# Enigmatisms/cvx_proj

Measured on AMD Instinct MI355X. Metric: local homographies/sec + Mpix/sec warp, 4K pair 200x200 mesh, higher is better.
Workload: dtype f64; 1 GPU; C3: 3840x2160 pair, 2000 correspondences, 200x200 mesh, canvas 4009x2242; mode=pairs, variant=auto, launch=eager, parallelism=pairsx1

## Files before the change

cvx_proj_amd/csrc/apap_kernels.hip:

```cpp
#include <hip/hip_runtime.h>

#include <cstdlib>
#include <type_traits>
#include <vector>

#include "apap_internal.h"
#include "apap_warp_dev.h"
#include "apap_weight_dev.h"

namespace {

using apap::inv3;
using apap::rcp_full;

using apap::kMoments;
constexpr int kWave = 64;

struct BatchStride {
    long long table, vertices, moments, denorm, H;
};


constexpr int kExpBits = 9;
constexpr int kExpN = 1 << kExpBits;
constexpr double kExpScale = (double)kExpN * 0x1.71547652b82fep+0;
__constant__ double kExp2Tab[kExpN] = {
    0x1.0000000000000p+0, 0x1.0058c86da1c0ap+0, 0x1.00b1afa5abcbfp+0, 0x1.010ab5b2cbd11p+0,
    0x1.0163da9fb3335p+0, 0x1.01bd1e77170b4p+0, 0x1.02168143b0281p+0, 0x1.027003103b10ep+0,
    0x1.02c9a3e778061p+0, 0x1.032363d42b027p+0, 0x1.037d42e11bbccp+0, 0x1.03d7411915a8ap+0,
    0x1.04315e86e7f85p+0, 0x1.048b9b35659d8p+0, 0x1.04e5f72f654b1p+0, 0x1.0540727fc1762p+0,
    0x1.059b0d3158574p+0, 0x1.05f5c74f0bec2p+0, 0x1.0650a0e3c1f89p+0, 0x1.06ab99fa6407cp+0,
    0x1.0706b29ddf6dep+0, 0x1.0761ead925493p+0, 0x1.07bd42b72a836p+0, 0x1.0818ba42e7d30p+0,
    0x1.0874518759bc8p+0, 0x1.08d0088f8093fp+0, 0x1.092bdf66607e0p+0, 0x1.0987d61701716p+0,
    0x1.09e3ecac6f383p+0, 0x1.0a402331b9715p+0, 0x1.0a9c79b1f3919p+0, 0x1.0af8f03834e52p+0,
    0x1.0b5586cf9890fp+0, 0x1.0bb23d833d93fp+0, 0x1.0c0f145e46c85p+0, 0x1.0c6c0b6bdae53p+0,
    0x1.0cc922b7247f7p+0, 0x1.0d265a4b520bap+0, 0x1.0d83b23395decp+0, 0x1.0de12a7b26300p+0,
    0x1.0e3ec32d3d1a2p+0, 0x1.0e9c7c55189c6p+0, 0x1.0efa55fdfa9c5p+0, 0x1.0f58503328e6dp+0,
    0x1.0fb66affed31bp+0, 0x1.1014a66f951cep+0, 0x1.1073028d7233ep+0, 0x1.10d17f64d9ef1p+0,
    0x1.11301d0125b51p+0, 0x1.118edb6db2dc1p+0, 0x1.11edbab5e2ab6p+0, 0x1.124cbae51a5c8p+0,
    0x1.12abdc06c31ccp+0, 0x1.130b1e264a0e9p+0, 0x1.136a814f204abp+0, 0x1.13ca058cbae1ep+0,
    0x1.1429aaea92de0p+0, 0x1.1489717425438p+0, 0x1.14e95934f312ep+0, 0x1.154962388149ep+0,
    0x1.15a98c8a58e51p+0, 0x1.1609d83606e12p+0, 0x1.166a45471c3c2p+0, 0x1.16cad3c92df73p+0,
    0x1.172b83c7d517bp+0, 0x1.178c554eaea89p+0, 0x1.17ed48695bbc0p+0, 0x1.184e5d23816c9p+0,
    0x1.18af9388c8deap+0, 0x1.1910eba4df41fp+0, 0x1.1972658375d2fp+0, 0x1.19d4013041dc2p+0,
    0x1.1a35beb6fcb75p+0, 0x1.1a979e2363cf8p+0, 0x1.1af99f8138a1cp+0, 0x1.1b5bc2dc40bf0p+0,
    0x1.1bbe084045cd4p+0, 0x1.1c206fb91588fp+0, 0x1.1c82f95281c6bp+0, 0x1.1ce5a51860746p+0,
    0x1.1d4873168b9aap+0, 0x1.1dab6358e15e8p+0, 0x1.1e0e75eb44027p+0, 0x1.1e71aad999e82p+0,
    0x1.1ed5022fcd91dp+0, 0x1.1f387bf9cda38p+0, 0x1.1f9c18438ce4dp+0, 0x1.1fffd7190241ep+0,
    0x1.2063b88628cd6p+0, 0x1.20c7bc96ffc18p+0, 0x1.212be3578a819p+0, 0x1.21902cd3d09b9p+0,
    0x1.21f49917ddc96p+0, 0x1.2259282fc1f27p+0, 0x1.22bdda27912d1p+0, 0x1.2322af0b63bffp+0,
    0x1.2387a6e756238p+0, 0x1.23ecc1c78903ap+0, 0x1.2451ffb82140ap+0, 0x1.24b760c547f15p+0,
    0x1.251ce4fb2a63fp+0, 0x1.25828c65fa1ffp+0, 0x1.25e85711ece75p+0, 0x1.264e450b3cb82p+0,
    0x1.26b4565e27cddp+0, 0x1.271a8b16f0a30p+0, 0x1.2780e341ddf29p+0, 0x1.27e75eeb3ab98p+0,
    0x1.284dfe1f56381p+0, 0x1.28b4c0ea83f36p+0, 0x1.291ba7591bb70p+0, 0x1.2982b17779965p+0,
    0x1.29e9df51fdee1p+0, 0x1.2a5130f50d65cp+0, 0x1.2ab8a66d10f13p+0, 0x1.2b203fc675d1fp+0,
    0x1.2b87fd0dad990p+0, 0x1.2befde4f2e280p+0, 0x1.2c57e39771b2fp+0, 0x1.2cc00cf2f6c18p+0,
    0x1.2d285a6e4030bp+0, 0x1.2d90cc15d5346p+0, 0x1.2df961f641589p+0, 0x1.2e621c1c14833p+0,
    0x1.2ecafa93e2f56p+0, 0x1.2f33fd6a454d2p+0, 0x1.2f9d24abd886bp+0, 0x1.300670653dfe4p+0,
    0x1.306fe0a31b715p+0, 0x1.30d975721b004p+0, 0x1.31432edeeb2fdp+0, 0x1.31ad0cf63eeacp+0,
    0x1.32170fc4cd831p+0, 0x1.3281375752b40p+0, 0x1.32eb83ba8ea32p+0, 0x1.3355f4fb45e20p+0,
    0x1.33c08b26416ffp+0, 0x1.342b46484ebb4p+0, 0x1.3496266e3fa2dp+0, 0x1.35012ba4ea77dp+0,
    0x1.356c55f929ff1p+0, 0x1.35d7a577dd72bp+0, 0x1.36431a2de883bp+0, 0x1.36aeb428335b4p+0,
    0x1.371a7373aa9cbp+0, 0x1.3786581d3f669p+0, 0x1.37f26231e754ap+0, 0x1.385e91be9c811p+0,
    0x1.38cae6d05d866p+0, 0x1.393761742d808p+0, 0x1.39a401b7140efp+0, 0x1.3a10c7a61d55bp+0,
    0x1.3a7db34e59ff7p+0, 0x1.3aeac4bcdf3eap+0, 0x1.3b57fbfec6cf4p+0, 0x1.3bc559212ef89p+0,
    0x1.3c32dc313a8e5p+0, 0x1.3ca0853c10f28p+0, 0x1.3d0e544ede173p+0, 0x1.3d7c4976d27fap+0,
    0x1.3dea64c123422p+0, 0x1.3e58a63b0a09bp+0, 0x1.3ec70df1c5175p+0, 0x1.3f359bf29743fp+0,
    0x1.3fa4504ac801cp+0, 0x1.40132b07a35dfp+0, 0x1.40822c367a024p+0, 0x1.40f153e4a136ap+0,
    0x1.4160a21f72e2ap+0, 0x1.41d016f44d8f5p+0, 0x1.423fb2709468ap+0, 0x1.42af74a1af3f1p+0,
    0x1.431f5d950a897p+0, 0x1.438f6d5817663p+0, 0x1.43ffa3f84b9d4p+0, 0x1.4470018321a1ap+0,
    0x1.44e086061892dp+0, 0x1.4551318eb43ecp+0, 0x1.45c2042a7d232p+0, 0x1.4632fde7006f4p+0,
    0x1.46a41ed1d0057p+0, 0x1.471566f8827d0p+0, 0x1.4786d668b3237p+0, 0x1.47f86d3001fe5p+0,
    0x1.486a2b5c13cd0p+0, 0x1.48dc10fa920a1p+0, 0x1.494e1e192aed2p+0, 0x1.49c052c5916c4p+0,
    0x1.4a32af0d7d3dep+0, 0x1.4aa532feaada6p+0, 0x1.4b17dea6db7d7p+0, 0x1.4b8ab213d5283p+0,
    0x1.4bfdad5362a27p+0, 0x1.4c70d073537cap+0, 0x1.4ce41b817c114p+0, 0x1.4d578e8bb586bp+0,
    0x1.4dcb299fddd0dp+0, 0x1.4e3eeccbd7b2ap+0, 0x1.4eb2d81d8abffp+0, 0x1.4f26eba2e35f0p+0,
    0x1.4f9b2769d2ca7p+0, 0x1.500f8b804f127p+0, 0x1.508417f4531eep+0, 0x1.50f8ccd3deb0dp+0,
    0x1.516daa2cf6642p+0, 0x1.51e2b00da3b14p+0, 0x1.5257de83f4eefp+0, 0x1.52cd359dfd53dp+0,
    0x1.5342b569d4f82p+0, 0x1.53b85df598d78p+0, 0x1.542e2f4f6ad27p+0, 0x1.54a4298571b06p+0,
    0x1.551a4ca5d920fp+0, 0x1.559098bed1bdfp+0, 0x1.56070dde910d2p+0, 0x1.567dac1351819p+0,
    0x1.56f4736b527dap+0, 0x1.576b63f4d854cp+0, 0x1.57e27dbe2c4cfp+0, 0x1.5859c0d59ca07p+0,
    0x1.58d12d497c7fdp+0, 0x1.5948c32824135p+0, 0x1.59c0827ff07ccp+0, 0x1.5a386b5f43d92p+0,
    0x1.5ab07dd485429p+0, 0x1.5b28b9ee20d1ep+0, 0x1.5ba11fba87a03p+0, 0x1.5c19af482fc8fp+0,
    0x1.5c9268a5946b7p+0, 0x1.5d0b4be135accp+0, 0x1.5d84590998b93p+0, 0x1.5dfd902d47c65p+0,
    0x1.5e76f15ad2148p+0, 0x1.5ef07ca0cbf0fp+0, 0x1.5f6a320dceb71p+0, 0x1.5fe411b078d26p+0,
    0x1.605e1b976dc09p+0, 0x1.60d84fd15612ap+0, 0x1.6152ae6cdf6f4p+0, 0x1.61cd3778bc944p+0,
    0x1.6247eb03a5585p+0, 0x1.62c2c91c56acdp+0, 0x1.633dd1d1929fdp+0, 0x1.63b90532205d8p+0,
    0x1.6434634ccc320p+0, 0x1.64afec30678b7p+0, 0x1.652b9febc8fb7p+0, 0x1.65a77e8dcc390p+0,
    0x1.6623882552225p+0, 0x1.669fbcc140be7p+0, 0x1.671c1c70833f6p+0, 0x1.6798a7420a036p+0,
    0x1.68155d44ca973p+0, 0x1.68923e87bfb7ap+0, 0x1.690f4b19e9538p+0, 0x1.698c830a4c8d4p+0,
    0x1.6a09e667f3bcdp+0, 0x1.6a877541ee718p+0, 0x1.6b052fa75173ep+0, 0x1.6b8315a736c75p+0,
    0x1.6c012750bdabfp+0, 0x1.6c7f64b30aa09p+0, 0x1.6cfdcddd47645p+0, 0x1.6d7c62dea2f8ap+0,
    0x1.6dfb23c651a2fp+0, 0x1.6e7a10a38cee8p+0, 0x1.6ef9298593ae5p+0, 0x1.6f786e7ba9fefp+0,
    0x1.6ff7df9519484p+0, 0x1.70777ce1303f6p+0, 0x1.70f7466f42e87p+0, 0x1.71773c4eaa988p+0,
    0x1.71f75e8ec5f74p+0, 0x1.7277ad3ef9011p+0, 0x1.72f8286ead08ap+0, 0x1.7378d02d50b8fp+0,
    0x1.73f9a48a58174p+0, 0x1.747aa5953c849p+0, 0x1.74fbd35d7cbfdp+0, 0x1.757d2df29ce7cp+0,
    0x1.75feb564267c9p+0, 0x1.768069c1a861dp+0, 0x1.77024b1ab6e09p+0, 0x1.7784597eeba8fp+0,
    0x1.780694fde5d3fp+0, 0x1.7888fda749e5dp+0, 0x1.790b938ac1cf6p+0, 0x1.798e56b7fcf03p+0,
    0x1.7a11473eb0187p+0, 0x1.7a94652e958aap+0, 0x1.7b17b0976cfdbp+0, 0x1.7b9b2988fb9ecp+0,
    0x1.7c1ed0130c132p+0, 0x1.7ca2a4456e7a3p+0, 0x1.7d26a62ff86f0p+0, 0x1.7daad5e2850acp+0,
    0x1.7e2f336cf4e62p+0, 0x1.7eb3bedf2e1b9p+0, 0x1.7f3878491c491p+0, 0x1.7fbd5fbab091fp+0,
    0x1.80427543e1a12p+0, 0x1.80c7b8f4abaa9p+0, 0x1.814d2add106d9p+0, 0x1.81d2cb0d1736ap+0,
    0x1.82589994cce13p+0, 0x1.82de968443d9ap+0, 0x1.8364c1eb941f7p+0, 0x1.83eb1bdadb46dp+0,
    0x1.8471a4623c7adp+0, 0x1.84f85b91e07f1p+0, 0x1.857f4179f5b21p+0, 0x1.8606562ab00ecp+0,
    0x1.868d99b4492edp+0, 0x1.87150c27004c2p+0, 0x1.879cad931a436p+0, 0x1.88247e08e1957p+0,
    0x1.88ac7d98a6699p+0, 0x1.8934ac52be8f7p+0, 0x1.89bd0a478580fp+0, 0x1.8a4597875c644p+0,
    0x1.8ace5422aa0dbp+0, 0x1.8b574029db01ep+0, 0x1.8be05bad61778p+0, 0x1.8c69a6bdb5598p+0,
    0x1.8cf3216b5448cp+0, 0x1.8d7ccbc6c19e6p+0, 0x1.8e06a5e0866d9p+0, 0x1.8e90afc931857p+0,
    0x1.8f1ae99157736p+0, 0x1.8fa553499284bp+0, 0x1.902fed0282c8ap+0, 0x1.90bab6ccce12cp+0,
    0x1.9145b0b91ffc6p+0, 0x1.91d0dad829e70p+0, 0x1.925c353aa2fe2p+0, 0x1.92e7bff148396p+0,
    0x1.93737b0cdc5e5p+0, 0x1.93ff669e2802bp+0, 0x1.948b82b5f98e5p+0, 0x1.9517cf65253d1p+0,
    0x1.95a44cbc8520fp+0, 0x1.9630faccf9243p+0, 0x1.96bdd9a7670b3p+0, 0x1.974ae95cba768p+0,
    0x1.97d829fde4e50p+0, 0x1.98659b9bddb5bp+0, 0x1.98f33e47a22a2p+0, 0x1.9981121235681p+0,
    0x1.9a0f170ca07bap+0, 0x1.9a9d4d47f2598p+0, 0x1.9b2bb4d53fe0dp+0, 0x1.9bba4dc5a3dd3p+0,
    0x1.9c49182a3f090p+0, 0x1.9cd81414380f2p+0, 0x1.9d674194bb8d5p+0, 0x1.9df6a0bcfc15ep+0,
    0x1.9e86319e32323p+0, 0x1.9f15f4499c647p+0, 0x1.9fa5e8d07f29ep+0, 0x1.a0360f4424fcbp+0,
    0x1.a0c667b5de565p+0, 0x1.a156f23701b15p+0, 0x1.a1e7aed8eb8bbp+0, 0x1.a2789dacfe68cp+0,
    0x1.a309bec4a2d33p+0, 0x1.a39b1231475f7p+0, 0x1.a42c980460ad8p+0, 0x1.a4be504f696b1p+0,
    0x1.a5503b23e255dp+0, 0x1.a5e25893523d4p+0, 0x1.a674a8af46052p+0, 0x1.a7072b8950a73p+0,
    0x1.a799e1330b358p+0, 0x1.a82cc9be14dcap+0, 0x1.a8bfe53c12e59p+0, 0x1.a95333beb0b7ep+0,
    0x1.a9e6b5579fdbfp+0, 0x1.aa7a6a1897fd2p+0, 0x1.ab0e521356ebap+0, 0x1.aba26d59a09eep+0,
    0x1.ac36bbfd3f37ap+0, 0x1.accb3e100301ep+0, 0x1.ad5ff3a3c2774p+0, 0x1.adf4dcca5a413p+0,
    0x1.ae89f995ad3adp+0, 0x1.af1f4a17a4735p+0, 0x1.afb4ce622f2ffp+0, 0x1.b04a868742ee4p+0,
    0x1.b0e07298db666p+0, 0x1.b17692a8fa8cdp+0, 0x1.b20ce6c9a8952p+0, 0x1.b2a36f0cf3f3ap+0,
    0x1.b33a2b84f15fbp+0, 0x1.b3d11c43bbd62p+0, 0x1.b468415b749b1p+0, 0x1.b4ff9ade433c6p+0,
    0x1.b59728de5593ap+0, 0x1.b62eeb6ddfc87p+0, 0x1.b6c6e29f1c52ap+0, 0x1.b75f0e844bfc6p+0,
    0x1.b7f76f2fb5e47p+0, 0x1.b89004b3a7804p+0, 0x1.b928cf22749e4p+0, 0x1.b9c1ce8e77680p+0,
    0x1.ba5b030a1064ap+0, 0x1.baf46ca7a67a7p+0, 0x1.bb8e0b79a6f1fp+0, 0x1.bc27df9285775p+0,
    0x1.bcc1e904bc1d2p+0, 0x1.bd5c27e2cb5e5p+0, 0x1.bdf69c3f3a207p+0, 0x1.be91462c95b60p+0,
    0x1.bf2c25bd71e09p+0, 0x1.bfc73b0468d30p+0, 0x1.c06286141b33dp+0, 0x1.c0fe06ff301f4p+0,
    0x1.c199bdd85529cp+0, 0x1.c235aab23e61ep+0, 0x1.c2d1cd9fa652cp+0, 0x1.c36e26b34e065p+0,
    0x1.c40ab5fffd07ap+0, 0x1.c4a77b9881650p+0, 0x1.c544778fafb22p+0, 0x1.c5e1a9f8630adp+0,
    0x1.c67f12e57d14bp+0, 0x1.c71cb269e601fp+0, 0x1.c7ba88988c933p+0, 0x1.c8589584661a1p+0,
    0x1.c8f6d9406e7b5p+0, 0x1.c99553dfa8313p+0, 0x1.ca3405751c4dbp+0, 0x1.cad2ee13da7cbp+0,
    0x1.cb720dcef9069p+0, 0x1.cc1164b994d23p+0, 0x1.ccb0f2e6d1675p+0, 0x1.cd50b869d8f0fp+0,
    0x1.cdf0b555dc3fap+0, 0x1.ce90e9be12cb9p+0, 0x1.cf3155b5bab74p+0, 0x1.cfd1f95018d17p+0,
    0x1.d072d4a07897cp+0, 0x1.d113e7ba2c38cp+0, 0x1.d1b532b08c968p+0, 0x1.d256b596f948cp+0,
    0x1.d2f87080d89f2p+0, 0x1.d39a638197a3cp+0, 0x1.d43c8eacaa1d6p+0, 0x1.d4def2158a91fp+0,
    0x1.d5818dcfba487p+0, 0x1.d62461eec14bep+0, 0x1.d6c76e862e6d3p+0, 0x1.d76ab3a99745bp+0,
    0x1.d80e316c98398p+0, 0x1.d8b1e7e2d479dp+0, 0x1.d955d71ff6075p+0, 0x1.d9f9ff37adb4ap+0,
    0x1.da9e603db3285p+0, 0x1.db42fa45c4dfdp+0, 0x1.dbe7cd63a8315p+0, 0x1.dc8cd9ab294e4p+0,
    0x1.dd321f301b460p+0, 0x1.ddd79e065807dp+0, 0x1.de7d5641c0658p+0, 0x1.df2347f63c159p+0,
    0x1.dfc97337b9b5fp+0, 0x1.e06fd81a2ece1p+0, 0x1.e11676b197d17p+0, 0x1.e1bd4f11f8220p+0,
    0x1.e264614f5a129p+0, 0x1.e30bad7dcee90p+0, 0x1.e3b333b16ee12p+0, 0x1.e45af3fe592e8p+0,
    0x1.e502ee78b3ff6p+0, 0x1.e5ab2334ac7eep+0, 0x1.e653924676d76p+0, 0x1.e6fc3bc24e350p+0,
    0x1.e7a51fbc74c83p+0, 0x1.e84e3e4933c7ep+0, 0x1.e8f7977cdb740p+0, 0x1.e9a12b6bc3181p+0,
    0x1.ea4afa2a490dap+0, 0x1.eaf503ccd2be5p+0, 0x1.eb9f4867cca6ep+0, 0x1.ec49c80faa594p+0,
    0x1.ecf482d8e67f1p+0, 0x1.ed9f78d802dc2p+0, 0x1.ee4aaa2188510p+0, 0x1.eef616ca06dd6p+0,
    0x1.efa1bee615a27p+0, 0x1.f04da28a52e59p+0, 0x1.f0f9c1cb6412ap+0, 0x1.f1a61cbdf5be7p+0,
    0x1.f252b376bba97p+0, 0x1.f2ff860a70c22p+0, 0x1.f3ac948dd7274p+0, 0x1.f459df15b82acp+0,
    0x1.f50765b6e4540p+0, 0x1.f5b5288633625p+0, 0x1.f6632798844f8p+0, 0x1.f7116302bd526p+0,
    0x1.f7bfdad9cbe14p+0, 0x1.f86e8f32a4b45p+0, 0x1.f91d802243c89p+0, 0x1.f9ccadbdac61dp+0,
    0x1.fa7c1819e90d8p+0, 0x1.fb2bbf4c0ba54p+0, 0x1.fbdba3692d514p+0, 0x1.fc8bc4866e8adp+0,
    0x1.fd3c22b8f71f1p+0, 0x1.fdecbe15f6314p+0, 0x1.fe9d96b2a23d9p+0, 0x1.ff4eaca4391b6p+0};

__device__ __forceinline__ double exp_neg_scaled(double yu, const double *tab ) {
    constexpr double L = 0x1.62e42fefa39efp-1 / kExpN;
    const int nk = (int)(-yu);
    const double f = __builtin_amdgcn_fract(yu);
    const double t = tab[nk & (kExpN - 1)];
    double p = fma(f, L * L * L * L / 24, -(L * L * L / 6));
    p = fma(f, p, L * L / 2);
    p = fma(f, p, -L);
    p = fma(f, p, 1.0);
    return __builtin_ldexp(t * p, nk >> kExpBits);
}

__device__ __forceinline__ double cell_weight_sq_tab(double vx, double vy, double sx, double sy,
                                                     double scaled_inv_sigma2, double gamma2, const double *tab) {
    const double dx = vx - sx;
    const double dy = vy - sy;
    const double x = fma(dx, dx, fma(dy, dy, 1e-300));
    const double y = __builtin_amdgcn_rsq(x);
    double g = x * y;
    const double e = fma(-g, y, 1.0);
    const double c = fma(e, 0.375, 0.5);
    g = fma(g * e, c, g);
    return fmax(exp_neg_scaled(g * scaled_inv_sigma2, tab), gamma2);
}

__device__ __forceinline__ double cell_weight_sq_f32(float vx, float vy, float2 s, float neg_scale, float gamma2) {
    const float dx = vx - s.x;
    const float dy = vy - s.y;
    const float d = __builtin_amdgcn_sqrtf(__builtin_fmaf(dx, dx, dy * dy));
    return (double)fmaxf(__builtin_amdgcn_exp2f(d * neg_scale), gamma2);
}

constexpr double kGammaCutF64 = 0x1p128;
__host__ __device__ inline double k1_gamma2(double gamma, bool w32) {
    if (gamma >= (w32 ? 1.0 : kGammaCutF64)) return 1.0;
    return gamma > 0.0 ? gamma * gamma : 0.0;
}

constexpr double kTraceFloorF64 = 1e-280;
constexpr double kTraceFloorW32 = 0x1p-40;

constexpr long long kTable24Marker = 0x7ff8242424242424ll;
__device__ __forceinline__ bool table_is_24(const double *__restrict__ table) {
    return __double_as_longlong(table[28]) == kTable24Marker;
}

typedef double double4_t __attribute__((ext_vector_type(4)));
constexpr int kChunk = 64;
static_assert(kChunk % 16 == 0 && kChunk % 4 == 0, "chunk must split evenly over 256 threads and 4-keypoint steps");

struct K1Block {
    int p_begin, p_end, nchunks;
    __device__ __forceinline__ K1Block(const double *__restrict__ &table, const double *__restrict__ &vertices,
                                       const BatchStride &bs, int n, int split, int pts_per_split) {
        table += (long long)blockIdx.z * bs.table;
        vertices += (long long)blockIdx.z * bs.vertices;
        p_begin = min(n, split * pts_per_split);
        p_end = min(n, p_begin + pts_per_split);
        nchunks = (p_end - p_begin + kChunk - 1) / kChunk;
    }
};

__device__ __forceinline__ double2 cell_vertex(const double *__restrict__ vertices, int cell, int cells) {
    const int cc = min(cell, cells - 1);
    return make_double2(vertices[2 * cc], vertices[2 * cc + 1]);
}

template <int kThreads>
__device__ __forceinline__ void exp_table_copy(double *s_exp2, int tid) {
    for (int j = tid; j < kExpN; j += kThreads) s_exp2[j] = kExp2Tab[j];
}
template <int kThreads>
struct ExpTableStage {
    static_assert(kExpN % kThreads == 0 || kThreads % kExpN == 0, "exp table vs block size");
    static constexpr int kPerThread = (kExpN + kThreads - 1) / kThreads;
    double v[kPerThread];
    __device__ __forceinline__ void fetch(int tid) {
#pragma unroll
        for (int i = 0; i < kPerThread; ++i) v[i] = kExp2Tab[(tid + i * kThreads) & (kExpN - 1)];
    }
    __device__ __forceinline__ void publish(double *s_exp2, int tid) const {
#pragma unroll
        for (int i = 0; i < kPerThread; ++i) s_exp2[(tid + i * kThreads) & (kExpN - 1)] = v[i];
    }
};

__host__ __device__ constexpr int lds_off(int r, int c) { return r * 256 + ((c ^ ((r & 1) << 4)) << 3); }
#define APAP_LDS_PIECE_OFF(r, slot) ((r) * 256 + ((slot) ^ (((r) & 1) << 3)) * 16)
constexpr bool lds_swizzles_agree() {
    for (int r = 0; r < 2; ++r)
        for (int slot = 0; slot < 16; ++slot)
            if (APAP_LDS_PIECE_OFF(r, slot) != lds_off(r, 2 * slot) || APAP_LDS_PIECE_OFF(r, slot) + 8 != lds_off(r, 2 * slot + 1))
                return false;
    return true;
}
static_assert(lds_swizzles_agree(), "a staged piece lands where lds_off looks for its two columns, for both row parities");

template <int kThreads>
using ChunkStage = double2[kChunk * 16 / kThreads];
template <int kThreads>
__device__ __forceinline__ void chunk_load(ChunkStage<kThreads> &stage, const double *__restrict__ table, int tid, int first_row,
                                           int end_row) {
#pragma unroll
    for (int i = 0; i < kChunk * 16 / kThreads; ++i) {
        const int q = tid + kThreads * i;
        const int p = first_row + (q >> 4);
        stage[i] = (p < end_row) ? *reinterpret_cast<const double2 *>(table + (size_t)p * APAP_TABLE_STRIDE + 2 * (q & 15))
                                 : make_double2(0.0, 0.0);
    }
}
#define APAP_CHUNK_STORE(kThreads, buf, stage, tid)                                          \
    do {                                                                                     \
        _Pragma("unroll") for (int i_ = 0; i_ < kChunk * 16 / (kThreads); ++i_) {            \
            const int q_ = (tid) + (kThreads) * i_;                                          \
            const int r_ = q_ >> 4, slot_ = q_ & 15;                                         \
            *reinterpret_cast<double2 *>(&(buf)[APAP_LDS_PIECE_OFF(r_, slot_)]) = (stage)[i_]; \
        }                                                                                    \
    } while (0)

template <bool kW32>
struct CellWeight {
    static constexpr int kXyColumn = kW32 ? 29 : 30;
    using Xy = std::conditional_t<kW32, float2, double2>;
    double vx, vy, scaled_inv_sigma2, gamma2;
    float vxf, vyf, neg_scale_f, gamma2f;
    const double *exp2;
    __device__ __forceinline__ void set(double2 v, double inv_sigma2, double gamma2_, const double *s_exp2) {
        vx = v.x, vy = v.y;
        scaled_inv_sigma2 = inv_sigma2 * kExpScale;
        gamma2 = gamma2_;
        vxf = (float)vx, vyf = (float)vy;
        neg_scale_f = (float)(inv_sigma2 * -0x1.71547652b82fep+0), gamma2f = (float)gamma2;
        exp2 = s_exp2;
    }
    static __device__ __forceinline__ Xy read(const unsigned char *at) { return *reinterpret_cast<const Xy *>(at); }
    __device__ __forceinline__ double sq(Xy s) const {
        if constexpr (kW32) return cell_weight_sq_f32(vxf, vyf, s, neg_scale_f, gamma2f);
        else return cell_weight_sq_tab(vx, vy, s.x, s.y, scaled_inv_sigma2, gamma2, exp2);
    }
    __device__ __forceinline__ double sq(const unsigned char *at) const { return sq(read(at)); }
};

template <bool kM24>
struct Sums16 {
    double4_t acc0 = {0.0, 0.0, 0.0, 0.0}, acc1 = {0.0, 0.0, 0.0, 0.0};
    double acc_a = 0.0, acc_b = 0.0;
    __device__ __forceinline__ void step(double w2, const unsigned char *at0, const unsigned char *at1) {
        const double b0 = *reinterpret_cast<const double *>(at0);
        const double b1 = *reinterpret_cast<const double *>(at1);
        acc0 = __builtin_amdgcn_mfma_f64_16x16x4f64(w2, b0, acc0, 0, 0, 0);
        if constexpr (kM24) {
            acc_a = __builtin_amdgcn_mfma_f64_4x4x4f64(w2, b1, acc_a, 0, 0, 0);
            acc_b = __builtin_amdgcn_mfma_f64_4x4x4f64(w2, *reinterpret_cast<const double *>(at1 + 32), acc_b, 0, 0, 0);
        } else {
            acc1 = __builtin_amdgcn_mfma_f64_16x16x4f64(w2, b1, acc1, 0, 0, 0);
        }
    }
    __device__ __forceinline__ void step(double w2, double b0, double b1, double b1b) {
        acc0 = __builtin_amdgcn_mfma_f64_16x16x4f64(w2, b0, acc0, 0, 0, 0);
        if constexpr (kM24) {
            acc_a = __builtin_amdgcn_mfma_f64_4x4x4f64(w2, b1, acc_a, 0, 0, 0);
            acc_b = __builtin_amdgcn_mfma_f64_4x4x4f64(w2, b1b, acc_b, 0, 0, 0);
        } else {
            acc1 = __builtin_amdgcn_mfma_f64_16x16x4f64(w2, b1, acc1, 0, 0, 0);
        }
    }
};

struct K1Pairs {
    int pairs, splits, tiles;
};
__host__ __device__ inline void k1_unit(const K1Pairs &pp, int i, int &tile, int &split, bool &paired) {
    const int base = pp.pairs / pp.splits, rem = pp.pairs % pp.splits;
    paired = i < pp.pairs;
    if (paired) {
        split = i % pp.splits;
        tile = 2 * (i / pp.splits);
        return;
    }
    int k = i - pp.pairs;
    const int n1 = pp.tiles - 2 * (base + 1), n0 = pp.tiles - 2 * base;
    if (k < rem * n1) {
        split = k / n1;
        tile = 2 * (base + 1) + k % n1;
    } else {
        k -= rem * n1;
        split = rem + k / n0;
        tile = 2 * base + k % n0;
    }
}

__host__ __device__ constexpr int d16_cell(int lane, int i) { return (lane >> 4) + 4 * i; }
__host__ __device__ constexpr int d16_column(int lane) { return lane & 15; }
__host__ __device__ constexpr int d4_cell(int lane) { return 4 * ((lane >> 2) & 3) + (lane >> 4); }
__host__ __device__ constexpr int d4_column(int lane) { return lane & 3; }

constexpr int kLinePitch = 144;
constexpr int kLineStageBytes = 32 * kLinePitch;
__host__ __device__ constexpr int line_stage_off(int column, int cell) { return column * kLinePitch + cell * 8; }
__host__ __device__ constexpr int line_column(int lane, int j) { return 8 * j + (lane >> 3); }
__host__ __device__ constexpr int line_cell(int lane) { return 2 * (lane & 7); }
__host__ __device__ constexpr int line_stores(int sums) { return (sums + 7) / 8; }
template <int kSums>
constexpr bool line_layout_covers() {
    static_assert(kSums == 30 || kSums == 24, "the two tables");
    int staged[32][16] = {}, stored[32][16] = {};
    for (int lane = 0; lane < 64; ++lane) {
        for (int i = 0; i < 4; ++i) {
            ++staged[d16_column(lane)][d16_cell(lane, i)];
            if (kSums == 30) ++staged[16 + d16_column(lane)][d16_cell(lane, i)];
        }
        if (kSums == 24) {
            ++staged[16 + d4_column(lane)][d4_cell(lane)];
            ++staged[20 + d4_column(lane)][d4_cell(lane)];
        }
        for (int j = 0; j < line_stores(kSums); ++j) {
            const int c = line_column(lane, j);
            if (c >= 32 || line_cell(lane) + 1 >= 16 || line_stage_off(c, line_cell(lane)) % 16 != 0 ||
                line_stage_off(c, line_cell(lane) + 1) != line_stage_off(c, line_cell(lane)) + 8)
                return false;
            if (c < kSums) ++stored[c][line_cell(lane)], ++stored[c][line_cell(lane) + 1];
        }
    }
    for (int c = 0; c < 32; ++c)
        for (int cell = 0; cell < 16; ++cell)
            if (staged[c][cell] != (c < (kSums == 30 ? 32 : 24)) || stored[c][cell] != (c < kSums)) return false;
    return true;
}
static_assert(line_layout_covers<30>() && line_layout_covers<24>(),
              "the line layout stores every sum of a 16-cell group once, columns from kSums on never, from what the D layouts staged");
static_assert(kLinePitch % 16 == 0 && 16 * 8 <= kLinePitch && 4 * kLineStageBytes <= 2 * kChunk * 256,
              "16-byte reads of whole rows; four waves' stages fit the two chunk buffers");

typedef double double2_t __attribute__((ext_vector_type(2)));
__device__ __forceinline__ void slab_store_line(double *p, double2_t v) {
    asm volatile("global_store_dwordx4 %0, %1, off sc1\n\ts_nop 1" ::"v"(p), "v"(v) : "memory");
}

__global__ __launch_bounds__(256) void k_assemble_valu(const double *__restrict__ table, int n,
                                                       const double *__restrict__ vertices, int cells,
                                                       int cells_pad, double gamma2, double inv_sigma2,
                                                       int pts_per_split, double *__restrict__ moments,
                                                       BatchStride bs) {
    __shared__ double s_exp2[kExpN];
    exp_table_copy<256>(s_exp2, threadIdx.x);
    __syncthreads();
    table += (long long)blockIdx.z * bs.table;
    vertices += (long long)blockIdx.z * bs.vertices;
    moments += (long long)blockIdx.z * bs.moments;
    const int lane = threadIdx.x & 63;
    const int wave = __builtin_amdgcn_readfirstlane(threadIdx.x >> 6);
    const int cell = (blockIdx.x * 4 + wave) * kWave + lane;
    if (cell - lane >= cells_pad) return;
    const double2 v = cell_vertex(vertices, cell, cells);
    const double vx = v.x, vy = v.y;
    const int p0 = min(n, (int)blockIdx.y * pts_per_split);
    const int p1 = min(n, p0 + pts_per_split);
    const double scaled_inv_sigma2 = inv_sigma2 * kExpScale;

    double acc[kMoments];
#pragma unroll
    for (int j = 0; j < kMoments; ++j) acc[j] = 0.0;

    double sx = 0.0, sy = 0.0;
    if (p0 < p1) {
        sx = table[(size_t)p0 * APAP_TABLE_STRIDE + 30];
        sy = table[(size_t)p0 * APAP_TABLE_STRIDE + 31];
    }
    __builtin_amdgcn_s_waitcnt(0x0070);
    for (int p = p0; p < p1; ++p) {
        const double *__restrict__ row = table + (size_t)p * APAP_TABLE_STRIDE;
        const double *__restrict__ nxt = table + (size_t)min(p + 1, p1 - 1) * APAP_TABLE_STRIDE;
        const double nsx = nxt[30], nsy = nxt[31];
        double r[kMoments];
#pragma unroll
        for (int j = 0; j < kMoments; ++j) r[j] = row[j];
        __builtin_amdgcn_sched_barrier(0);
        const double w2 = cell_weight_sq_tab(vx, vy, sx, sy, scaled_inv_sigma2, gamma2, s_exp2);
#pragma unroll
        for (int j = 0; j < kMoments; ++j) acc[j] = fma(w2, r[j], acc[j]);
        __builtin_amdgcn_sched_barrier(0);
        sx = nsx;
        sy = nsy;
    }
    double *dst = moments + (size_t)blockIdx.y * kMoments * cells_pad + cell;
#pragma unroll
    for (int j = 0; j < kMoments; ++j) dst[(size_t)j * cells_pad] = acc[j];
}

template <int kWaves, bool kM24, bool kW32, int kGroups, bool kLevel>
__device__ __forceinline__ void k1_mfma_tiles(unsigned char (&lds)[2][kChunk * 256], double *s_exp2, const double *__restrict__ table,
                                              const double *__restrict__ vertices, int cells, int cells_pad, double gamma2,
                                              double inv_sigma2, double *__restrict__ slab, int tile, const K1Block &blk) {
    constexpr int kThreads = kWaves * 64;
    const int tid = threadIdx.x;
    ExpTableStage<kThreads> exp_stage;
    exp_stage.fetch(tid);
    const int lane = tid & 63;
    const int wave = tid >> 6;
    const int kgrp = lane >> 4;
    const int col = lane & 15;
    CellWeight<kW32> weight[kGroups];
#pragma unroll
    for (int t = 0; t < kGroups; ++t)
        weight[t].set(cell_vertex(vertices, (tile + t) * (16 * kWaves) + wave * 16 + col, cells), inv_sigma2, gamma2, s_exp2);
    const int p_begin = blk.p_begin, p_end = blk.p_end, nchunks = blk.nchunks;

    ChunkStage<kThreads> stage;
    const int off_xy = lds_off(kgrp, CellWeight<kW32>::kXyColumn), off_b0 = lds_off(kgrp, col);
    const int off_b1 = lds_off(kgrp, 16 + (kM24 ? (lane & 3) : col));
    Sums16<kM24> sums[kGroups];
    auto step2 = [&](const double (&w2)[kGroups], const unsigned char *at0, const unsigned char *at1) {
        const double b0 = *reinterpret_cast<const double *>(at0);
        const double b1 = *reinterpret_cast<const double *>(at1);
        const double b1b = kM24 ? *reinterpret_cast<const double *>(at1 + 32) : 0.0;
#pragma unroll
        for (int t = 0; t < kGroups; ++t) sums[t].step(w2[t], b0, b1, b1b);
    };
    if (nchunks > 0) chunk_load<kThreads>(stage, table, tid, p_begin, p_end);
    exp_stage.publish(s_exp2, tid);
    if (nchunks > 0) APAP_CHUNK_STORE(kThreads, lds[0], stage, tid);
    __syncthreads();
    __builtin_amdgcn_s_waitcnt(0x0070);
    const int nfull = (p_end - p_begin) / kChunk;
    for (int c = 0; c < nfull; ++c) {
        if constexpr (kLevel) {
            if (4 * c < nfull) __builtin_amdgcn_s_setprio(3);
            else if (4 * c < 2 * nfull) __builtin_amdgcn_s_setprio(2);
            else if (4 * c < 3 * nfull) __builtin_amdgcn_s_setprio(1);
            else __builtin_amdgcn_s_setprio(0);
        }
        if (c + 1 < nchunks) chunk_load<kThreads>(stage, table, tid, p_begin + (c + 1) * kChunk, p_end);
        const unsigned char *buf = lds[c & 1];
        if constexpr (kGroups == 1) {
#pragma unroll
            for (int s0 = 0; s0 < kChunk / 4; s0 += 8) {
                double w2[8];
#pragma unroll
                for (int g = 0; g < 8; ++g) w2[g] = weight[0].sq(buf + off_xy + 1024 * (s0 + g));
                __builtin_amdgcn_sched_barrier(0);
#pragma unroll
                for (int g = 0; g < 8; ++g) sums[0].step(w2[g], buf + off_b0 + 1024 * (s0 + g), buf + off_b1 + 1024 * (s0 + g));
                __builtin_amdgcn_sched_barrier(0);
            }
        } else {
            constexpr int kSteps = kW32 ? 2 : 4;
#pragma unroll
            for (int s0 = 0; s0 < kChunk / 4; s0 += kSteps) {
                double w2[kSteps][kGroups];
#pragma unroll
                for (int g = 0; g < kSteps; ++g) {
                    const auto xy = CellWeight<kW32>::read(buf + off_xy + 1024 * (s0 + g));
#pragma unroll
                    for (int t = 0; t < kGroups; ++t) w2[g][t] = weight[t].sq(xy);
                }
                __builtin_amdgcn_sched_barrier(0);
#pragma unroll
                for (int g = 0; g < kSteps; ++g) step2(w2[g], buf + off_b0 + 1024 * (s0 + g), buf + off_b1 + 1024 * (s0 + g));
                __builtin_amdgcn_sched_barrier(0);
            }
        }
        if (c + 1 < nchunks) APAP_CHUNK_STORE(kThreads, lds[(c + 1) & 1], stage, tid);
        __syncthreads();
    }
    if (nfull < nchunks) {
        const unsigned char *buf = lds[nfull & 1];
        const int steps_here = (p_end - p_begin - nfull * kChunk + 3) >> 2;
        for (int s1 = 0; s1 < steps_here; ++s1) {
            if constexpr (kGroups == 1) {
                sums[0].step(weight[0].sq(buf + off_xy + 1024 * s1), buf + off_b0 + 1024 * s1, buf + off_b1 + 1024 * s1);
            } else {
                const auto xy = CellWeight<kW32>::read(buf + off_xy + 1024 * s1);
                double w2[kGroups];
#pragma unroll
                for (int t = 0; t < kGroups; ++t) w2[t] = weight[t].sq(xy);
                step2(w2, buf + off_b0 + 1024 * s1, buf + off_b1 + 1024 * s1);
            }
        }
        __syncthreads();
    }

    static_assert(kWaves * kLineStageBytes <= (int)sizeof(lds), "a stage per wave");
    constexpr int kSums = kM24 ? 24 : kMoments;
    const int wave_u = __builtin_amdgcn_readfirstlane(wave);
    unsigned char *stage_lds = &lds[0][0] + wave_u * kLineStageBytes;
#pragma unroll
    for (int t = 0; t < kGroups; ++t) {
        const int cell_base = (tile + t) * (16 * kWaves) + wave_u * 16;
        if (t > 0) {
            __builtin_amdgcn_fence(__ATOMIC_RELEASE, "wavefront");
            __builtin_amdgcn_wave_barrier();
            __builtin_amdgcn_fence(__ATOMIC_ACQUIRE, "wavefront");
        }
#pragma unroll
        for (int i = 0; i < 4; ++i) {
            *reinterpret_cast<double *>(stage_lds + line_stage_off(d16_column(lane), d16_cell(lane, i))) = sums[t].acc0[i];
            if constexpr (!kM24)
                *reinterpret_cast<double *>(stage_lds + line_stage_off(16 + d16_column(lane), d16_cell(lane, i))) = sums[t].acc1[i];
        }
        if constexpr (kM24) {
            *reinterpret_cast<double *>(stage_lds + line_stage_off(16 + d4_column(lane), d4_cell(lane))) = sums[t].acc_a;
            *reinterpret_cast<double *>(stage_lds + line_stage_off(20 + d4_column(lane), d4_cell(lane))) = sums[t].acc_b;
        }
        __builtin_amdgcn_fence(__ATOMIC_RELEASE, "wavefront");
        __builtin_amdgcn_wave_barrier();
        __builtin_amdgcn_fence(__ATOMIC_ACQUIRE, "wavefront");
        if (cell_base < cells_pad) {
#pragma unroll
            for (int j = 0; j < line_stores(kSums); ++j) {
                const int c = line_column(lane, j);
                const double2_t v = *reinterpret_cast<const double2_t *>(stage_lds + line_stage_off(c, line_cell(lane)));
                if (c < kSums) slab_store_line(slab + (size_t)c * cells_pad + cell_base + line_cell(lane), v);
            }
        }
    }
}

template <int kWaves, bool kM24, bool kW32>
__global__ __launch_bounds__(kWaves * 64) void k_assemble_mfma(const double *__restrict__ table, int n,
                                                       const double *__restrict__ vertices, int cells,
                                                       int cells_pad, double gamma2, double inv_sigma2,
                                                       int pts_per_split, double *__restrict__ moments,
                                                       BatchStride bs, K1Pairs pp) {
    __shared__ __attribute__((aligned(16))) unsigned char lds[2][kChunk * 256];
    __shared__ double s_exp2[kExpN];
    int tile = blockIdx.x, split = blockIdx.y;
    bool paired = false;
    if (pp.pairs > 0) k1_unit(pp, (int)blockIdx.x, tile, split, paired);
    const K1Block blk(table, vertices, bs, n, split, pts_per_split);
    constexpr int kSums = kM24 ? 24 : kMoments;
    double *slab = moments + (long long)blockIdx.z * bs.moments + (size_t)split * kSums * cells_pad;
    if (paired)
        k1_mfma_tiles<kWaves, kM24, kW32, 2, true>(lds, s_exp2, table, vertices, cells, cells_pad, gamma2, inv_sigma2, slab, tile, blk);
    else if (pp.pairs > 0)
        k1_mfma_tiles<kWaves, kM24, kW32, 1, true>(lds, s_exp2, table, vertices, cells, cells_pad, gamma2, inv_sigma2, slab, tile, blk);
    else
        k1_mfma_tiles<kWaves, kM24, kW32, 1, false>(lds, s_exp2, table, vertices, cells, cells_pad, gamma2, inv_sigma2, slab, tile, blk);
}

template <int kGroups, int kQuads, bool kW32>
__global__ __launch_bounds__(256) void k_assemble_mfma4(const double *__restrict__ table, int n,
                                                        const double *__restrict__ vertices, int cells,
                                                        int cells_pad, double gamma2, double inv_sigma2,
                                                        int pts_per_split, double *__restrict__ moments,
                                                        BatchStride bs) {
    __shared__ __attribute__((aligned(16))) unsigned char lds[2][kChunk * 256];
    const K1Block blk(table, vertices, bs, n, (int)blockIdx.y, pts_per_split);
    moments += (long long)blockIdx.z * bs.moments;
    __shared__ double s_exp2[kExpN];
    exp_table_copy<256>(s_exp2, threadIdx.x);
    const int tid = threadIdx.x;
    const int lane = tid & 63;
    const int wave = tid >> 6;
    const int kgrp = lane >> 4;
    const int col = lane & 15;
    const int cell0 = (blockIdx.x * 4 + wave) * (16 * kGroups);
    CellWeight<kW32> weight[kGroups];
#pragma unroll
    for (int g = 0; g < kGroups; ++g) weight[g].set(cell_vertex(vertices, cell0 + 16 * g + col, cells), inv_sigma2, gamma2, s_exp2);
    const int p_begin = blk.p_begin, p_end = blk.p_end, nchunks = blk.nchunks;

    ChunkStage<256> stage;
    const int off_xy = lds_off(kgrp, CellWeight<kW32>::kXyColumn);
    const int off_lo = lds_off(kgrp, lane & 3), off_hi = lds_off(kgrp, 16 + (lane & 3));
    double acc[kGroups][kQuads];
#pragma unroll
    for (int g = 0; g < kGroups; ++g)
#pragma unroll
        for (int m = 0; m < kQuads; ++m) acc[g][m] = 0.0;
    if (nchunks > 0) {
        chunk_load<256>(stage, table, tid, p_begin, p_end);
        APAP_CHUNK_STORE(256, lds[0], stage, tid);
    }
    __syncthreads();
    __builtin_amdgcn_s_waitcnt(0x0070);
    for (int c = 0; c < nchunks; ++c) {
        if (c + 1 < nchunks) chunk_load<256>(stage, table, tid, p_begin + (c + 1) * kChunk, p_end);
        const unsigned char *buf = lds[c & 1];
#pragma unroll
        for (int s = 0; s < kChunk / 4; ++s) {
            double bv[kQuads];
#pragma unroll
            for (int m = 0; m < kQuads; ++m)
                bv[m] = *reinterpret_cast<const double *>(buf + (m < 4 ? off_lo : off_hi) + 32 * (m & 3) + 1024 * s);
            double w2[kGroups];
            const auto xy = CellWeight<kW32>::read(buf + off_xy + 1024 * s);
#pragma unroll
            for (int g = 0; g < kGroups; ++g) w2[g] = weight[g].sq(xy);
#pragma unroll
            for (int m = 0; m < kQuads; ++m)
#pragma unroll
                for (int g = 0; g < kGroups; ++g)
                    acc[g][m] = __builtin_amdgcn_mfma_f64_4x4x4f64(w2[g], bv[m], acc[g][m], 0, 0, 0);
        }
        if (c + 1 < nchunks) APAP_CHUNK_STORE(256, lds[(c + 1) & 1], stage, tid);
        __syncthreads();
    }
    constexpr int kSums = kQuads == 6 ? 24 : kMoments;
    double *slab = moments + (size_t)blockIdx.y * kSums * cells_pad;
    const int dcell = d4_cell(lane);
    const int dj = d4_column(lane);
#pragma unroll
    for (int g = 0; g < kGroups; ++g) {
        const int ci = cell0 + 16 * g + dcell;
        if (ci < cells_pad) {
#pragma unroll
            for (int m = 0; m < kQuads; ++m)
                if (4 * m + dj < kSums) slab[(size_t)(4 * m + dj) * cells_pad + ci] = acc[g][m];
        }
    }
}

__host__ __device__ constexpr int tri(int i, int j) {
    return i <= j ? i * (19 - i) / 2 + (j - i) : j * (19 - j) / 2 + (i - j);
}

template <int P, int Q>
__device__ __forceinline__ void jacobi_rotate(double (&a)[45], double (&v)[81]) {
    const double apq = a[tri(P, Q)];
    const double app = a[tri(P, P)];
    const double aqq = a[tri(Q, Q)];
    const double theta = 0.5 * (aqq - app) / apq;
    double t = copysign(1.0, theta) / (fabs(theta) + sqrt(fma(theta, theta, 1.0)));
    t = (apq != 0.0) ? t : 0.0;
    const double c = 1.0 / sqrt(fma(t, t, 1.0));
    const double s = t * c;
    a[tri(P, P)] = fma(-t, apq, app);
    a[tri(Q, Q)] = fma(t, apq, aqq);
    a[tri(P, Q)] = 0.0;
#pragma unroll
    for (int k = 0; k < 9; ++k) {
        if (k != P && k != Q) {
            const double akp = a[tri(k, P)];
            const double akq = a[tri(k, Q)];
            a[tri(k, P)] = fma(c, akp, -(s * akq));
            a[tri(k, Q)] = fma(s, akp, c * akq);
        }
    }
#pragma unroll
    for (int k = 0; k < 9; ++k) {
        const double vkp = v[9 * k + P];
        const double vkq = v[9 * k + Q];
        v[9 * k + P] = fma(c, vkp, -(s * vkq));
        v[9 * k + Q] = fma(s, vkp, c * vkq);
    }
}

__device__ __forceinline__ void jacobi_sweep(double (&a)[45], double (&v)[81]) {
#define APAP_ROW(p, q) jacobi_rotate<p, q>(a, v);
    APAP_ROW(0, 1) APAP_ROW(0, 2) APAP_ROW(0, 3) APAP_ROW(0, 4) APAP_ROW(0, 5) APAP_ROW(0, 6) APAP_ROW(0, 7) APAP_ROW(0, 8)
    APAP_ROW(1, 2) APAP_ROW(1, 3) APAP_ROW(1, 4) APAP_ROW(1, 5) APAP_ROW(1, 6) APAP_ROW(1, 7) APAP_ROW(1, 8)
    APAP_ROW(2, 3) APAP_ROW(2, 4) APAP_ROW(2, 5) APAP_ROW(2, 6) APAP_ROW(2, 7) APAP_ROW(2, 8)
    APAP_ROW(3, 4) APAP_ROW(3, 5) APAP_ROW(3, 6) APAP_ROW(3, 7) APAP_ROW(3, 8)
    APAP_ROW(4, 5) APAP_ROW(4, 6) APAP_ROW(4, 7) APAP_ROW(4, 8)
    APAP_ROW(5, 6) APAP_ROW(5, 7) APAP_ROW(5, 8)
    APAP_ROW(6, 7) APAP_ROW(6, 8)
    APAP_ROW(7, 8)
#undef APAP_ROW
}

__device__ __forceinline__ void mul3(const double *x, const double *y, double *out) {
#pragma unroll
    for (int i = 0; i < 3; ++i)
#pragma unroll
        for (int j = 0; j < 3; ++j)
            out[3 * i + j] = fma(x[3 * i + 2], y[6 + j], fma(x[3 * i + 1], y[3 + j], x[3 * i] * y[j]));
}

constexpr int kMaxSweeps = 15;

__device__ __forceinline__ double jacobi_eigvec(double (&a)[45], int pick_rank, double (&h)[9]) {
    double v[81];
#pragma unroll
    for (int k = 0; k < 81; ++k) v[k] = (k % 10 == 0) ? 1.0 : 0.0;
    for (int sweep = 0; sweep < kMaxSweeps; ++sweep) {
        jacobi_sweep(a, v);
        double off2 = 0.0, trace = 0.0;
#pragma unroll
        for (int i = 0; i < 9; ++i) {
            trace += fabs(a[tri(i, i)]);
#pragma unroll
            for (int j = i + 1; j < 9; ++j) off2 = fma(a[tri(i, j)], a[tri(i, j)], off2);
        }
        const bool done = off2 <= 1e-34 * trace * trace;
        if (__all(done)) break;
    }
    int best = 0;
    double lam0 = 0.0, lam1 = 0.0;
#pragma unroll
    for (int i = 0; i < 9; ++i) {
// ... 1901 lines not shown
```

Measured before the change: 278.9 million homographies/s.

## Share per-row dy² term across cells in the f64 MFMA assembly kernel

A tile of mesh cells spans at most two distinct vertex rows (y values). When that holds, owner threads now compute (vy - sy)^2 once per keypoint and row and publish it to a small double-buffered LDS side table. Each cell then only computes dx^2 and adds the shared term, which saves one subtract and one FMA per weight in the f64 path. In exchange the kernel pays for extra LDS reads and writes, a row-detection prologue using ballot/readlane, an extra global load per chunk for owner threads, and a duplicated code path that raises instruction footprint and register pressure.

```diff
diff --git a/cvx_proj_amd/csrc/apap_kernels.hip b/cvx_proj_amd/csrc/apap_kernels.hip
--- a/cvx_proj_amd/csrc/apap_kernels.hip
+++ b/cvx_proj_amd/csrc/apap_kernels.hip
@@ -5,6 +5,7 @@
 #include <vector>
 
 #include "apap_internal.h"
+#include "apap_row_term.h"
 #include "apap_warp_dev.h"
 #include "apap_weight_dev.h"
 
@@ -166,17 +167,24 @@
     return __builtin_ldexp(t * p, nk >> kExpBits);
 }
 
-__device__ __forceinline__ double cell_weight_sq_tab(double vx, double vy, double sx, double sy,
-                                                     double scaled_inv_sigma2, double gamma2, const double *tab) {
-    const double dx = vx - sx;
-    const double dy = vy - sy;
-    const double x = fma(dx, dx, fma(dy, dy, 1e-300));
+__device__ __forceinline__ double cell_weight_sq_of(double x, double scaled_inv_sigma2, double gamma2, const double *tab) {
     const double y = __builtin_amdgcn_rsq(x);
     double g = x * y;
     const double e = fma(-g, y, 1.0);
     const double c = fma(e, 0.375, 0.5);
     g = fma(g * e, c, g);
     return fmax(exp_neg_scaled(g * scaled_inv_sigma2, tab), gamma2);
+}
+__device__ __forceinline__ double cell_weight_sq_tab(double vx, double vy, double sx, double sy,
+                                                     double scaled_inv_sigma2, double gamma2, const double *tab) {
+    const double dx = vx - sx;
+    const double dy = vy - sy;
+    return cell_weight_sq_of(fma(dx, dx, fma(dy, dy, 1e-300)), scaled_inv_sigma2, gamma2, tab);
+}
+__device__ __forceinline__ double cell_weight_sq_row(double vx, double sx, double row_term,
+                                                     double scaled_inv_sigma2, double gamma2, const double *tab) {
+    const double dx = vx - sx;
+    return cell_weight_sq_of(fma(dx, dx, row_term), scaled_inv_sigma2, gamma2, tab);
 }
 
 __device__ __forceinline__ double cell_weight_sq_f32(float vx, float vy, float2 s, float neg_scale, float gamma2) {
@@ -294,6 +302,9 @@
         else return cell_weight_sq_tab(vx, vy, s.x, s.y, scaled_inv_sigma2, gamma2, exp2);
     }
     __device__ __forceinline__ double sq(const unsigned char *at) const { return sq(read(at)); }
+    __device__ __forceinline__ double sq_row(double sx, double row_term) const {
+        return cell_weight_sq_row(vx, sx, row_term, scaled_inv_sigma2, gamma2, exp2);
+    }
 };
 
 template <bool kM24>
@@ -444,9 +455,10 @@
 }
 
 template <int kWaves, bool kM24, bool kW32, int kGroups, bool kLevel>
-__device__ __forceinline__ void k1_mfma_tiles(unsigned char (&lds)[2][kChunk * 256], double *s_exp2, const double *__restrict__ table,
-                                              const double *__restrict__ vertices, int cells, int cells_pad, double gamma2,
-                                              double inv_sigma2, double *__restrict__ slab, int tile, const K1Block &blk) {
+__device__ __forceinline__ void k1_mfma_tiles(unsigned char (&lds)[2][kChunk * 256], double *s_exp2, double (&s_row)[2][kChunk][2],
+                                              const double *__restrict__ table, const double *__restrict__ vertices, int cells,
+                                              int cells_pad, double gamma2, double inv_sigma2, double *__restrict__ slab, int tile,
+                                              const K1Block &blk) {
     constexpr int kThreads = kWaves * 64;
     const int tid = threadIdx.x;
     ExpTableStage<kThreads> exp_stage;
@@ -461,6 +473,52 @@
         weight[t].set(cell_vertex(vertices, (tile + t) * (16 * kWaves) + wave * 16 + col, cells), inv_sigma2, gamma2, s_exp2);
     const int p_begin = blk.p_begin, p_end = blk.p_end, nchunks = blk.nchunks;
 
+    constexpr bool kCanShare = !kW32;
+    bool share = false;
+    double row_v = 0.0;
+    bool row_owner = false;
+    int off_row[kGroups];
+    if constexpr (kCanShare) {
+        static_assert(kWaves == 4 && kThreads >= apap::kRowOwners && kChunk == apap::kRowChunk, "the side table's owners");
+        const int first = tile * (16 * kWaves);
+        auto uniform_bits = [](double v) {
+            const long long b = __double_as_longlong(v);
+            return (long long)(((unsigned long long)(unsigned)__builtin_amdgcn_readfirstlane((int)(b >> 32)) << 32) |
+                               (unsigned)__builtin_amdgcn_readfirstlane((int)b));
+        };
+        const long long a_bits = uniform_bits(cell_vertex(vertices, first, cells).y);
+        long long seen[kGroups];
+#pragma unroll
+        for (int t = 0; t < kGroups; ++t) seen[t] = __double_as_longlong(cell_vertex(vertices, first + 64 * t + lane, cells).y);
+        long long b_bits = a_bits;
+#pragma unroll
+        for (int t = kGroups - 1; t >= 0; --t) {
+            const unsigned long long other = __ballot(seen[t] != a_bits);
+            const int l = other ? __builtin_ctzll(other) : 0;
+            const long long there = (long long)(((unsigned long long)(unsigned)__builtin_amdgcn_readlane((int)(seen[t] >> 32), l) << 32) |
+                                                (unsigned)__builtin_amdgcn_readlane((int)seen[t], l));
+            b_bits = other ? there : b_bits;
+        }
+        bool mine = true;
+#pragma unroll
+        for (int t = 0; t < kGroups; ++t) mine = mine && apap::row_is_shared(seen[t], a_bits, b_bits);
+        share = __all(mine);
+        const int wave_r = __builtin_amdgcn_readfirstlane(wave);
+        row_owner = wave_r < apap::kRowOwners / 64;
+        row_v = __longlong_as_double(apap::row_owner_value(wave_r * 64) == 0 ? a_bits : b_bits);
+#pragma unroll
+        for (int t = 0; t < kGroups; ++t)
+            off_row[t] = apap::row_read_off(0, 0, kgrp, apap::row_value(__double_as_longlong(weight[t].vy), a_bits));
+    }
+    auto row_fetch = [&](int first_row) {
+        const int p = first_row + apap::row_owner_keypoint(tid);
+        return p < p_end ? table[(size_t)p * APAP_TABLE_STRIDE + 31] : 0.0;
+    };
+    auto row_publish = [&](int buffer, double sy) {
+        const double dy = row_v - sy;
+        s_row[buffer][apap::row_owner_keypoint(tid)][apap::row_owner_value(tid)] = fma(dy, dy, 1e-300);
+    };
+
     ChunkStage<kThreads> stage;
     const int off_xy = lds_off(kgrp, CellWeight<kW32>::kXyColumn), off_b0 = lds_off(kgrp, col);
     const int off_b1 = lds_off(kgrp, 16 + (kM24 ? (lane & 3) : col));
@@ -473,66 +531,117 @@
         for (int t = 0; t < kGroups; ++t) sums[t].step(w2[t], b0, b1, b1b);
     };
     if (nchunks > 0) chunk_load<kThreads>(stage, table, tid, p_begin, p_end);
+    double row_y0 = 0.0;
+    if constexpr (kCanShare) {
+        if (row_owner && nchunks > 0) row_y0 = row_fetch(p_begin);
+    }
     exp_stage.publish(s_exp2, tid);
     if (nchunks > 0) APAP_CHUNK_STORE(kThreads, lds[0], stage, tid);
+    if constexpr (kCanShare) {
+        if (row_owner && nchunks > 0) row_publish(0, row_y0);
+    }
     __syncthreads();
     __builtin_amdgcn_s_waitcnt(0x0070);
     const int nfull = (p_end - p_begin) / kChunk;
-    for (int c = 0; c < nfull; ++c) {
-        if constexpr (kLevel) {
-            if (4 * c < nfull) __builtin_amdgcn_s_setprio(3);
-            else if (4 * c < 2 * nfull) __builtin_amdgcn_s_setprio(2);
-            else if (4 * c < 3 * nfull) __builtin_amdgcn_s_setprio(1);
-            else __builtin_amdgcn_s_setprio(0);
-        }
-        if (c + 1 < nchunks) chunk_load<kThreads>(stage, table, tid, p_begin + (c + 1) * kChunk, p_end);
-        const unsigned char *buf = lds[c & 1];
-        if constexpr (kGroups == 1) {
-#pragma unroll
-            for (int s0 = 0; s0 < kChunk / 4; s0 += 8) {
-                double w2[8];
-#pragma unroll
-                for (int g = 0; g < 8; ++g) w2[g] = weight[0].sq(buf + off_xy + 1024 * (s0 + g));
-                __builtin_amdgcn_sched_barrier(0);
-#pragma unroll
-                for (int g = 0; g < 8; ++g) sums[0].step(w2[g], buf + off_b0 + 1024 * (s0 + g), buf + off_b1 + 1024 * (s0 + g));
-                __builtin_amdgcn_sched_barrier(0);
+    auto chunks = [&](auto row_tag) {
+        constexpr bool kRow = decltype(row_tag)::value;
+        auto w2_row = [&](int t, double sx, const unsigned char *rbuf, int s) {
+            return weight[t].sq_row(sx, *reinterpret_cast<const double *>(rbuf + off_row[t] + apap::kRowStepBytes * s));
+        };
+        for (int c = 0; c < nfull; ++c) {
+            if constexpr (kLevel) {
+                if (4 * c < nfull) __builtin_amdgcn_s_setprio(3);
+                else if (4 * c < 2 * nfull) __builtin_amdgcn_s_setprio(2);
+                else if (4 * c < 3 * nfull) __builtin_amdgcn_s_setprio(1);
+                else __builtin_amdgcn_s_setprio(0);
             }
-        } else {
-            constexpr int kSteps = kW32 ? 2 : 4;
-#pragma unroll
-            for (int s0 = 0; s0 < kChunk / 4; s0 += kSteps) {
-                double w2[kSteps][kGroups];
-#pragma unroll
-                for (int g = 0; g < kSteps; ++g) {
-                    const auto xy = CellWeight<kW32>::read(buf + off_xy + 1024 * (s0 + g));
-#pragma unroll
-                    for (int t = 0; t < kGroups; ++t) w2[g][t] = weight[t].sq(xy);
+            ChunkStage<kThreads> next;
+            double row_y = 0.0;
+            if (c + 1 < nchunks) {
+                chunk_load<kThreads>(next, table, tid, p_begin + (c + 1) * kChunk, p_end);
+                if constexpr (kRow) {
+                    if (row_owner) row_y = row_fetch(p_begin + (c + 1) * kChunk);
                 }
-                __builtin_amdgcn_sched_barrier(0);
-#pragma unroll
-                for (int g = 0; g < kSteps; ++g) step2(w2[g], buf + off_b0 + 1024 * (s0 + g), buf + off_b1 + 1024 * (s0 + g));
-                __builtin_amdgcn_sched_barrier(0);
             }
-        }
-        if (c + 1 < nchunks) APAP_CHUNK_STORE(kThreads, lds[(c + 1) & 1], stage, tid);
-        __syncthreads();
-    }
-    if (nfull < nchunks) {
-        const unsigned char *buf = lds[nfull & 1];
-        const int steps_here = (p_end - p_begin - nfull * kChunk + 3) >> 2;
-        for (int s1 = 0; s1 < steps_here; ++s1) {
+            const unsigned char *buf = lds[c & 1];
+            const unsigned char *rbuf = reinterpret_cast<const unsigned char *>(s_row[c & 1]);
             if constexpr (kGroups == 1) {
-                sums[0].step(weight[0].sq(buf + off_xy + 1024 * s1), buf + off_b0 + 1024 * s1, buf + off_b1 + 1024 * s1);
+#pragma unroll
+                for (int s0 = 0; s0 < kChunk / 4; s0 += 8) {
+                    double w2[8];
+#pragma unroll
+                    for (int g = 0; g < 8; ++g) {
+                        if constexpr (kRow) w2[g] = w2_row(0, *reinterpret_cast<const double *>(buf + off_xy + 1024 * (s0 + g)), rbuf, s0 + g);
+                        else w2[g] = weight[0].sq(buf + off_xy + 1024 * (s0 + g));
+                    }
+                    __builtin_amdgcn_sched_barrier(0);
+#pragma unroll
+                    for (int g = 0; g < 8; ++g) sums[0].step(w2[g], buf + off_b0 + 1024 * (s0 + g), buf + off_b1 + 1024 * (s0 + g));
+                    __builtin_amdgcn_sched_barrier(0);
+                }
             } else {
-                const auto xy = CellWeight<kW32>::read(buf + off_xy + 1024 * s1);
-                double w2[kGroups];
-#pragma unroll
-                for (int t = 0; t < kGroups; ++t) w2[t] = weight[t].sq(xy);
-                step2(w2, buf + off_b0 + 1024 * s1, buf + off_b1 + 1024 * s1);
+                constexpr int kSteps = kW32 ? 2 : 4;
+#pragma unroll
+                for (int s0 = 0; s0 < kChunk / 4; s0 += kSteps) {
+                    double w2[kSteps][kGroups];
+#pragma unroll
+                    for (int g = 0; g < kSteps; ++g) {
+                        if constexpr (kRow) {
+                            const double sx = *reinterpret_cast<const double *>(buf + off_xy + 1024 * (s0 + g));
+#pragma unroll
+                            for (int t = 0; t < kGroups; ++t) w2[g][t] = w2_row(t, sx, rbuf, s0 + g);
+                        } else {
+                            const auto xy = CellWeight<kW32>::read(buf + off_xy + 1024 * (s0 + g));
+#pragma unroll
+                            for (int t = 0; t < kGroups; ++t) w2[g][t] = weight[t].sq(xy);
+                        }
+                    }
+                    __builtin_amdgcn_sched_barrier(0);
+#pragma unroll
+                    for (int g = 0; g < kSteps; ++g) step2(w2[g], buf + off_b0 + 1024 * (s0 + g), buf + off_b1 + 1024 * (s0 + g));
+                    __builtin_amdgcn_sched_barrier(0);
+                }
             }
-        }
-        __syncthreads();
+            if (c + 1 < nchunks) {
+                APAP_CHUNK_STORE(kThreads, lds[(c + 1) & 1], next, tid);
+                if constexpr (kRow) {
+                    if (row_owner) row_publish((c + 1) & 1, row_y);
+                }
+            }
+            __syncthreads();
+        }
+        if (nfull < nchunks) {
+            const unsigned char *buf = lds[nfull & 1];
+            const unsigned char *rbuf = reinterpret_cast<const unsigned char *>(s_row[nfull & 1]);
+            const int steps_here = (p_end - p_begin - nfull * kChunk + 3) >> 2;
+            for (int s1 = 0; s1 < steps_here; ++s1) {
+                if constexpr (kGroups == 1) {
+                    double w2;
+                    if constexpr (kRow) w2 = w2_row(0, *reinterpret_cast<const double *>(buf + off_xy + 1024 * s1), rbuf, s1);
+                    else w2 = weight[0].sq(buf + off_xy + 1024 * s1);
+                    sums[0].step(w2, buf + off_b0 + 1024 * s1, buf + off_b1 + 1024 * s1);
+                } else {
+                    double w2[kGroups];
+                    if constexpr (kRow) {
+                        const double sx = *reinterpret_cast<const double *>(buf + off_xy + 1024 * s1);
+#pragma unroll
+                        for (int t = 0; t < kGroups; ++t) w2[t] = w2_row(t, sx, rbuf, s1);
+                    } else {
+                        const auto xy = CellWeight<kW32>::read(buf + off_xy + 1024 * s1);
+#pragma unroll
+                        for (int t = 0; t < kGroups; ++t) w2[t] = weight[t].sq(xy);
+                    }
+                    step2(w2, buf + off_b0 + 1024 * s1, buf + off_b1 + 1024 * s1);
+                }
+            }
+            __syncthreads();
+        }
+    };
+    if constexpr (kCanShare) {
+        if (share) chunks(std::true_type{});
+        else chunks(std::false_type{});
+    } else {
+        chunks(std::false_type{});
     }
 
     static_assert(kWaves * kLineStageBytes <= (int)sizeof(lds), "a stage per wave");
@@ -579,6 +688,7 @@
                                                        BatchStride bs, K1Pairs pp) {
     __shared__ __attribute__((aligned(16))) unsigned char lds[2][kChunk * 256];
     __shared__ double s_exp2[kExpN];
+    __shared__ __attribute__((aligned(16))) double s_row[2][kChunk][2];
     int tile = blockIdx.x, split = blockIdx.y;
     bool paired = false;
     if (pp.pairs > 0) k1_unit(pp, (int)blockIdx.x, tile, split, paired);
@@ -586,11 +696,11 @@
     constexpr int kSums = kM24 ? 24 : kMoments;
     double *slab = moments + (long long)blockIdx.z * bs.moments + (size_t)split * kSums * cells_pad;
     if (paired)
-        k1_mfma_tiles<kWaves, kM24, kW32, 2, true>(lds, s_exp2, table, vertices, cells, cells_pad, gamma2, inv_sigma2, slab, tile, blk);
+        k1_mfma_tiles<kWaves, kM24, kW32, 2, true>(lds, s_exp2, s_row, table, vertices, cells, cells_pad, gamma2, inv_sigma2, slab, tile, blk);
     else if (pp.pairs > 0)
-        k1_mfma_tiles<kWaves, kM24, kW32, 1, true>(lds, s_exp2, table, vertices, cells, cells_pad, gamma2, inv_sigma2, slab, tile, blk);
+        k1_mfma_tiles<kWaves, kM24, kW32, 1, true>(lds, s_exp2, s_row, table, vertices, cells, cells_pad, gamma2, inv_sigma2, slab, tile, blk);
     else
-        k1_mfma_tiles<kWaves, kM24, kW32, 1, false>(lds, s_exp2, table, vertices, cells, cells_pad, gamma2, inv_sigma2, slab, tile, blk);
+        k1_mfma_tiles<kWaves, kM24, kW32, 1, false>(lds, s_exp2, s_row, table, vertices, cells, cells_pad, gamma2, inv_sigma2, slab, tile, blk);
 }
 
 template <int kGroups, int kQuads, bool kW32>
diff --git a/cvx_proj_amd/csrc/apap_row_term.h b/cvx_proj_amd/csrc/apap_row_term.h
--- /dev/null
+++ b/cvx_proj_amd/csrc/apap_row_term.h
@@ -0,0 +1,33 @@
+#pragma once
+
+#if defined(__HIP__)
+#define APAP_ROW_HD __host__ __device__
+#else
+#define APAP_ROW_HD
+#endif
+
+namespace apap {
+
+constexpr int kRowChunk = 64;
+constexpr int kRowOwners = 2 * kRowChunk;
+constexpr int kRowBytes = 2 * kRowChunk * 2 * 8;
+
+APAP_ROW_HD constexpr long long row_second_value(const long long *bits, int n) {
+    for (int i = 1; i < n; ++i)
+        if (bits[i] != bits[0]) return bits[i];
+    return bits[0];
+}
+APAP_ROW_HD constexpr bool row_is_shared(long long vy_bits, long long a_bits, long long b_bits) {
+    return vy_bits == a_bits || vy_bits == b_bits;
+}
+APAP_ROW_HD constexpr int row_value(long long vy_bits, long long a_bits) { return vy_bits == a_bits ? 0 : 1; }
+
+APAP_ROW_HD constexpr int row_term_off(int buffer, int keypoint, int value) { return (buffer * kRowChunk + keypoint) * 16 + value * 8; }
+APAP_ROW_HD constexpr int row_owner_keypoint(int t) { return t & (kRowChunk - 1); }
+APAP_ROW_HD constexpr int row_owner_value(int t) { return t / kRowChunk; }
+constexpr int kRowStepBytes = 4 * 16;
+APAP_ROW_HD constexpr int row_read_off(int buffer, int step, int kgrp, int value) {
+    return row_term_off(buffer, 0, 0) + row_term_off(0, kgrp, value) + step * kRowStepBytes;
+}
+
+}
```

Measured after the change: 284.4 million homographies/s (median of 6 runs). +2.0%, better.
